# customink/lambdipy

Measured on NVIDIA H100. Metric: ELF-strip GB/s (build-tree .so bytes), higher is better.
Workload: dtype u8

## Files before the change

include/lambdipy_b200.h:

```cpp
#ifndef LAMBDIPY_B200_H
#define LAMBDIPY_B200_H
#include <stdint.h>
#ifdef __cplusplus
extern "C" {
#endif

typedef struct lb2_ctx lb2_ctx;

enum {
  LB2_OK = 0,
  LB2_E_CUDA = -1,
  LB2_E_ARG = -2,
  LB2_E_CAPACITY = -3,
  LB2_E_IO = -4,
  LB2_E_NODEVICE = -5,
  LB2_E_STATE = -6
};

enum {
  LB2_ST_OK = 0,
  LB2_ST_NOT_ELF = 1,
  LB2_ST_NOT_ELF64LE = 2,
  LB2_ST_BAD_TYPE = 3,
  LB2_ST_NO_SECTIONS = 4,
  LB2_ST_XINDEX = 5,
  LB2_ST_UNSUPPORTED_LAYOUT = 6,
  LB2_ST_BAD_NOTES = 7,
  LB2_ST_PLANNER_LIMIT = 8,
  LB2_ST_MALFORMED = -1
};

#define LB2_F_NO_MERGE_NOTES 1u

#define LB2_TREE_FALLBACK_HOST_STRIP 0x100u
#define LB2_TREE_TOLERATE_NON_ELF    0x200u
#define LB2_TREE_DRY_RUN             0x400u
#define LB2_TREE_CLEANUP             0x800u

typedef struct lb2_stats {
  uint32_t n_files, n_ok, n_unsupported, overflow;
  uint64_t in_bytes;
  uint64_t out_bytes;
  uint64_t copy_bytes;
  uint64_t header_bytes;
  uint64_t n_tiles;
  uint64_t out_bytes_needed;
  float plan_ms;
  float compact_ms;
  float h2d_ms, d2h_ms;
  uint64_t h2d_bytes;
  uint64_t d2h_bytes;
} lb2_stats;

typedef struct lb2_tree_stats {
  uint32_t n_selected;
  uint32_t n_gpu;
  uint32_t n_fallback;
  uint32_t n_skipped;
  uint32_t n_failed;
  uint32_t n_removed;
  uint64_t in_bytes, out_bytes;
  double walk_read_s;
  double gpu_s;
  double write_s;
  double fallback_s;
  double read_cpu_s;
  double write_cpu_s;
  double dma_wait_s;
  uint32_t io_threads, n_batches;
  lb2_stats batch;
} lb2_tree_stats;

int lb2_ctx_create(int device, lb2_ctx **ctx);
void lb2_ctx_destroy(lb2_ctx *ctx);
const char *lb2_last_error(const lb2_ctx *ctx);
const char *lb2_version(void);
int lb2_sm_count(const lb2_ctx *ctx);

void *lb2_dev_alloc(lb2_ctx *ctx, uint64_t bytes);
void lb2_dev_free(lb2_ctx *ctx, void *p);
void *lb2_pinned_alloc(lb2_ctx *ctx, uint64_t bytes);
void lb2_pinned_free(lb2_ctx *ctx, void *p);
int lb2_memcpy_h2d(lb2_ctx *ctx, void *d_dst, const void *h_src, uint64_t bytes);
int lb2_memcpy_d2h(lb2_ctx *ctx, void *h_dst, const void *d_src, uint64_t bytes);
int lb2_memset_d(lb2_ctx *ctx, void *d_dst, int value, uint64_t bytes);

int lb2_strip_device_async(lb2_ctx *ctx, const void *d_in, const uint64_t *h_in_off, const uint64_t *h_in_sizes,
                           uint32_t n_files, void *d_out, uint64_t out_capacity, uint32_t flags, void *stream);
int lb2_batch_results(lb2_ctx *ctx, uint64_t *h_out_off , uint64_t *h_out_sizes ,
                      int32_t *h_status , lb2_stats *stats);

typedef int (*lb2_chunk_fn)(void *user, uint32_t chunk, uint32_t first_file, uint32_t n_files, const void *d_out_slot,
                            const uint64_t *out_off, const uint64_t *out_sizes, const int32_t *status,
                            const lb2_stats *chunk_stats);
int lb2_strip_device_chunked(lb2_ctx *ctx, const void *d_in, const uint64_t *h_in_off, const uint64_t *h_in_sizes,
                             uint32_t n_files, void *d_out_ring, uint64_t slot_capacity, uint64_t max_chunk_bytes,
                             uint32_t flags, void *stream, lb2_chunk_fn on_chunk, void *user, uint64_t *h_out_sizes,
                             int32_t *h_status, lb2_stats *total);

int lb2_strip_host(lb2_ctx *ctx, const void *h_in, const uint64_t *h_in_off, const uint64_t *h_in_sizes,
                   uint32_t n_files, void *h_out, uint64_t out_capacity, uint64_t *h_out_off, uint64_t *h_out_sizes,
                   int32_t *h_status, uint32_t flags, lb2_stats *stats);

int lb2_strip_tree(lb2_ctx *ctx, const char *root, const char *suffix , uint32_t flags,
                   lb2_tree_stats *stats);
int lb2_strip_tree_ex(lb2_ctx *ctx, const char *root, const char *suffix, uint32_t flags, const char *keep_tests_regex,
                      lb2_tree_stats *stats);
int lb2_tree_cleanup(const char *root, const char *keep_tests_regex, uint32_t *n_removed);
int lb2_tree_prepare(lb2_ctx *ctx, uint64_t expected_tree_bytes);

int lb2_plan_device(lb2_ctx *ctx, const void *d_in, const uint64_t *h_in_off, const uint64_t *h_in_sizes,
                    uint32_t n_files, uint32_t flags, uint64_t *h_out_sizes, int32_t *h_status, lb2_stats *stats);

typedef struct lb2_fill_region {
  uint64_t offset;
  uint64_t len;
} lb2_fill_region;
int lb2_corpus_fill(lb2_ctx *ctx, void *d_arena, const lb2_fill_region *h_regions, uint32_t n_regions,
                    uint64_t seed, void *stream);

int lb2_corpus_scatter(lb2_ctx *ctx, void *d_arena, const void *h_data, uint64_t data_bytes, const uint64_t *h_dst,
                       const uint64_t *h_src, const uint64_t *h_len, uint32_t n);

#ifdef __cplusplus
}
#endif
#endif
```

lambdipy_b200/_native.py:

```python
import ctypes as C
import os

_HERE = os.path.dirname(os.path.abspath(__file__))
LIB_PATH = os.environ.get("LAMBDIPY_B200_LIB") or os.path.join(_HERE, "liblambdipy_b200.so")

LB2_OK, LB2_E_CUDA, LB2_E_ARG, LB2_E_CAPACITY, LB2_E_IO, LB2_E_NODEVICE, LB2_E_STATE = 0, -1, -2, -3, -4, -5, -6
ST_OK, ST_NOT_ELF, ST_NOT_ELF64LE, ST_BAD_TYPE, ST_NO_SECTIONS, ST_XINDEX = 0, 1, 2, 3, 4, 5
ST_UNSUPPORTED_LAYOUT, ST_BAD_NOTES, ST_PLANNER_LIMIT, ST_MALFORMED = 6, 7, 8, -1
F_NO_MERGE_NOTES = 1
TREE_FALLBACK_HOST_STRIP, TREE_TOLERATE_NON_ELF, TREE_DRY_RUN, TREE_CLEANUP = 0x100, 0x200, 0x400, 0x800

EXPORTS = [
    "lb2_ctx_create", "lb2_ctx_destroy", "lb2_last_error", "lb2_version", "lb2_sm_count",
    "lb2_dev_alloc", "lb2_dev_free", "lb2_pinned_alloc", "lb2_pinned_free",
    "lb2_memcpy_h2d", "lb2_memcpy_d2h", "lb2_memset_d",
    "lb2_strip_device_async", "lb2_batch_results", "lb2_strip_host", "lb2_strip_tree",
    "lb2_plan_device", "lb2_corpus_fill", "lb2_corpus_scatter",
    "lb2_strip_device_chunked", "lb2_tree_prepare", "lb2_strip_tree_ex", "lb2_tree_cleanup",
]


class Stats(C.Structure):
    _fields_ = [
        ("n_files", C.c_uint32), ("n_ok", C.c_uint32), ("n_unsupported", C.c_uint32), ("overflow", C.c_uint32),
        ("in_bytes", C.c_uint64), ("out_bytes", C.c_uint64), ("copy_bytes", C.c_uint64), ("header_bytes", C.c_uint64),
        ("n_tiles", C.c_uint64), ("out_bytes_needed", C.c_uint64),
        ("plan_ms", C.c_float), ("compact_ms", C.c_float), ("h2d_ms", C.c_float), ("d2h_ms", C.c_float),
        ("h2d_bytes", C.c_uint64), ("d2h_bytes", C.c_uint64),
    ]

    def as_dict(self):
        return {k: getattr(self, k) for k, _ in self._fields_}


class TreeStats(C.Structure):
    _fields_ = [
        ("n_selected", C.c_uint32), ("n_gpu", C.c_uint32), ("n_fallback", C.c_uint32), ("n_skipped", C.c_uint32),
        ("n_failed", C.c_uint32), ("n_removed", C.c_uint32),
        ("in_bytes", C.c_uint64), ("out_bytes", C.c_uint64),
        ("walk_read_s", C.c_double), ("gpu_s", C.c_double), ("write_s", C.c_double), ("fallback_s", C.c_double),
        ("read_cpu_s", C.c_double), ("write_cpu_s", C.c_double), ("dma_wait_s", C.c_double), ("io_threads", C.c_uint32), ("n_batches", C.c_uint32),
        ("batch", Stats),
    ]

    def as_dict(self):
        d = {k: getattr(self, k) for k, _ in self._fields_ if k != "batch"}
        d["batch"] = self.batch.as_dict()
        return d


class FillRegion(C.Structure):
    _fields_ = [("offset", C.c_uint64), ("len", C.c_uint64)]


class NativeError(RuntimeError):
    def __init__(self, code, msg):
        super().__init__("lambdipy_b200: rc=%d: %s" % (code, msg))
        self.code = code


class NoDeviceError(NativeError):
    pass


_lib = None


def load():
    global _lib
    if _lib is not None:
        return _lib
    if not os.path.exists(LIB_PATH):
        raise ImportError("%s is missing: run `python -m lambdipy_b200.build` (needs nvcc); "
                          "there is no CPU fallback for the strip path" % LIB_PATH)
    lib = C.CDLL(LIB_PATH)
    vp, u64p, i32p = C.c_void_p, C.POINTER(C.c_uint64), C.POINTER(C.c_int32)
    lib.lb2_ctx_create.argtypes = [C.c_int, C.POINTER(vp)]
    lib.lb2_ctx_create.restype = C.c_int
    lib.lb2_ctx_destroy.argtypes = [vp]
    lib.lb2_ctx_destroy.restype = None
    lib.lb2_last_error.argtypes = [vp]
    lib.lb2_last_error.restype = C.c_char_p
    lib.lb2_version.restype = C.c_char_p
    lib.lb2_sm_count.argtypes = [vp]
    lib.lb2_sm_count.restype = C.c_int
    lib.lb2_dev_alloc.argtypes = [vp, C.c_uint64]
    lib.lb2_dev_alloc.restype = vp
    lib.lb2_dev_free.argtypes = [vp, vp]
    lib.lb2_dev_free.restype = None
    lib.lb2_pinned_alloc.argtypes = [vp, C.c_uint64]
    lib.lb2_pinned_alloc.restype = vp
    lib.lb2_pinned_free.argtypes = [vp, vp]
    lib.lb2_pinned_free.restype = None
    lib.lb2_memcpy_h2d.argtypes = [vp, vp, vp, C.c_uint64]
    lib.lb2_memcpy_h2d.restype = C.c_int
    lib.lb2_memcpy_d2h.argtypes = [vp, vp, vp, C.c_uint64]
    lib.lb2_memcpy_d2h.restype = C.c_int
    lib.lb2_memset_d.argtypes = [vp, vp, C.c_int, C.c_uint64]
    lib.lb2_memset_d.restype = C.c_int
    lib.lb2_strip_device_async.argtypes = [vp, vp, u64p, u64p, C.c_uint32, vp, C.c_uint64, C.c_uint32, vp]
    lib.lb2_strip_device_async.restype = C.c_int
    lib.lb2_batch_results.argtypes = [vp, u64p, u64p, i32p, C.POINTER(Stats)]
    lib.lb2_batch_results.restype = C.c_int
    lib.lb2_strip_host.argtypes = [vp, vp, u64p, u64p, C.c_uint32, vp, C.c_uint64, u64p, u64p, i32p, C.c_uint32,
                                   C.POINTER(Stats)]
    lib.lb2_strip_host.restype = C.c_int
    lib.lb2_strip_tree.argtypes = [vp, C.c_char_p, C.c_char_p, C.c_uint32, C.POINTER(TreeStats)]
    lib.lb2_strip_tree.restype = C.c_int
    lib.lb2_plan_device.argtypes = [vp, vp, u64p, u64p, C.c_uint32, C.c_uint32, u64p, i32p, C.POINTER(Stats)]
    lib.lb2_plan_device.restype = C.c_int
    lib.lb2_corpus_fill.argtypes = [vp, vp, C.POINTER(FillRegion), C.c_uint32, C.c_uint64, vp]
    lib.lb2_corpus_fill.restype = C.c_int
    lib.lb2_corpus_scatter.argtypes = [vp, vp, vp, C.c_uint64, u64p, u64p, u64p, C.c_uint32]
    lib.lb2_corpus_scatter.restype = C.c_int
    lib.lb2_strip_device_chunked.argtypes = [vp, vp, u64p, u64p, C.c_uint32, vp, C.c_uint64, C.c_uint64, C.c_uint32, vp,
                                             vp, vp, u64p, i32p, C.POINTER(Stats)]
    lib.lb2_strip_device_chunked.restype = C.c_int
    lib.lb2_strip_tree_ex.argtypes = [vp, C.c_char_p, C.c_char_p, C.c_uint32, C.c_char_p, C.POINTER(TreeStats)]
    lib.lb2_strip_tree_ex.restype = C.c_int
    lib.lb2_tree_cleanup.argtypes = [C.c_char_p, C.c_char_p, C.POINTER(C.c_uint32)]
    lib.lb2_tree_cleanup.restype = C.c_int
    lib.lb2_tree_prepare.argtypes = [vp, C.c_uint64]
    lib.lb2_tree_prepare.restype = C.c_int
    _lib = lib
    return lib
# ... 67 lines not shown
```

lambdipy_b200/build.py:

```python
import os
import subprocess
import sys

HERE = os.path.dirname(os.path.abspath(__file__))
CSRC = os.path.join(HERE, "csrc")
OUT = os.path.join(HERE, "liblambdipy_b200.so")
SOURCES = ["plan.cu", "compact.cu", "compact_tma.cu", "corpus.cu", "api.cu"]
HEADERS = ["lb2_common.cuh", "copy_device.cuh", os.path.join("..", "..", "include", "lambdipy_b200.h")]
NVCC_FLAGS = [
    "-gencode", "arch=compute_90a,code=sm_90a", "-lineinfo", "-O3", "-std=c++17",
    "-Xcompiler", "-fPIC,-Wall,-Wno-unused-function", "--shared", "-cudart", "shared",
]


def needs_build():
    if not os.path.exists(OUT):
        return True
    t = os.path.getmtime(OUT)
    deps = [os.path.join(CSRC, s) for s in SOURCES + HEADERS] + [os.path.abspath(__file__)]
    return any(os.path.getmtime(d) > t for d in deps)


TIMING_OUT = os.path.join(HERE, "liblambdipy_b200_timing.so")


def build(force=False, verbose=False, timing=False):
    out = TIMING_OUT if timing else OUT
    if not timing and not force and not needs_build():
        return OUT
    nvcc = os.environ.get("NVCC", "/usr/local/cuda/bin/nvcc")
    cmd = [nvcc] + NVCC_FLAGS + (["-DLB2_PLAN_TIMING"] if timing else []) + (["-Xptxas", "-v"] if verbose else []) + \
        ["-o", out] + [os.path.join(CSRC, s) for s in SOURCES]
    r = subprocess.run(cmd, capture_output=True, text=True)
    if r.returncode != 0:
        sys.stderr.write(r.stdout + r.stderr)
        raise RuntimeError("nvcc failed building liblambdipy_b200.so")
    if verbose:
        sys.stderr.write(r.stdout + r.stderr)
    return out


if __name__ == "__main__":
    print(build(force="--force" in sys.argv, verbose="-v" in sys.argv, timing="--timing" in sys.argv))
```

lambdipy_b200/csrc/api.cu:

```cuda
#include "lb2_common.cuh"
#include "../../include/lambdipy_b200.h"

#include <algorithm>
#include <atomic>
#include <chrono>
#include <cctype>
#include <cerrno>
#include <cstdio>
#include <cstdlib>
#include <condition_variable>
#include <cstring>
#include <mutex>
#include <string>
#include <thread>
#include <vector>

#include <climits>
#include <dirent.h>
#include <regex.h>
#include <fcntl.h>
#include <spawn.h>
#include <sys/stat.h>
#include <sys/syscall.h>
#include <sys/wait.h>
// ... 767 lines not shown
    rmdir(p.c_str());
  } else {
    unlink(p.c_str());
  }
}

static void walk(const std::string &dir, const std::string &shown, bool top, const char *suffix, Cleanup *cl,
                 std::vector<TreeFile> &files, lb2_tree_stats *st) {
  DIR *d = opendir(dir.c_str());
  if (!d) return;
  std::vector<std::string> names;
  while (dirent *e = readdir(d))
    if (strcmp(e->d_name, ".") && strcmp(e->d_name, "..")) names.push_back(e->d_name);
  closedir(d);
  for (const std::string &name : names) {
    const std::string p = dir + "/" + name, line = shown + name;
    struct stat lsb, sb;
    if (lstat(p.c_str(), &lsb) != 0) continue;
    if (cl && cl->on) {
      bool remove = false;
      if (top && name[0] != '.' && (ends_with(name.c_str(), ".egg-info") || ends_with(name.c_str(), ".dist-info"))) remove = true;
      else if (name == "__pycache__") remove = true;
      else if (name == "tests" && line.find('\n') == std::string::npos &&
               !(cl->have_keep && regexec(&cl->keep, line.c_str(), 0, nullptr, 0) == 0)) remove = true;
      if (remove) { rm_rf(p); cl->n_removed++; continue; }
    }
    if (suffix && ends_with(name.c_str(), suffix)) {
      st->n_selected++;
      if (stat(p.c_str(), &sb) != 0 || !S_ISREG(sb.st_mode)) {
        st->n_failed++;
      } else {
        if (S_ISLNK(lsb.st_mode)) st->n_skipped++;
        files.push_back({p, (uint64_t)sb.st_size, sb.st_dev, sb.st_ino, 1});
      }
    }
    if (S_ISDIR(lsb.st_mode)) walk(p, line + "/", false, suffix, cl, files, st);
  }
}

static bool cleanup_init(Cleanup &cl, const char *keep_regex, std::string *err) {
  cl.on = true;
  if (keep_regex && *keep_regex) {
    if (regcomp(&cl.keep, keep_regex, REG_NOSUB) != 0) { if (err) *err = std::string("bad keep-tests pattern: ") + keep_regex; return false; }
    cl.have_keep = true;
  }
  return true;
}

static void dedupe(std::vector<TreeFile> &files) {
  std::sort(files.begin(), files.end(), [](const TreeFile &a, const TreeFile &b) {
    if (a.dev != b.dev) return a.dev < b.dev;
    if (a.ino != b.ino) return a.ino < b.ino;
    return a.path < b.path;
  });
  size_t w = 0;
  for (size_t i = 0; i < files.size(); i++) {
    if (w && files[w - 1].dev == files[i].dev && files[w - 1].ino == files[i].ino) files[w - 1].times++;
    else files[w++] = files[i];
  }
  files.resize(w);
  std::sort(files.begin(), files.end(), [](const TreeFile &a, const TreeFile &b) { return a.path < b.path; });
}

static int host_strip(const std::string &p) {
  const char *argv[] = {"strip", p.c_str(), nullptr};
  pid_t pid;
  if (posix_spawnp(&pid, "strip", nullptr, nullptr, const_cast<char *const *>(argv), environ) != 0) return 127;
  int status = 0;
  while (waitpid(pid, &status, 0) < 0 && errno == EINTR) {}
  return WIFEXITED(status) ? WEXITSTATUS(status) : 128;
}

template <class F> static void parallel_for(size_t n, int threads, F f) {
  std::atomic<size_t> next{0};
  std::vector<std::thread> pool;
  threads = (int)std::max<size_t>(1, std::min<size_t>((size_t)std::max(threads, 1), n));
  for (int t = 0; t < threads; t++)
    pool.emplace_back([&] { for (size_t i; (i = next.fetch_add(1)) < n;) f(i); });
  for (auto &th : pool) th.join();
}

struct Seg { uint32_t file; uint64_t file_off, len, slot_off; };
struct Slice { bool upload; uint8_t *dev; uint64_t len; uint32_t seg0, seg1; };

static void make_slices(bool upload, uint8_t *dev_base, const std::vector<uint32_t> &ids, const uint64_t *offs, const uint64_t *sizes,
                        uint64_t slot_bytes, std::vector<Seg> &segs, std::vector<Slice> &out) {
  const size_t m = ids.size();
  size_t k = 0;
  uint64_t c = 0;
  while (k < m) {
    if (sizes[k] == 0) { k++; c = 0; continue; }
    const uint64_t a = offs[k] + c, end = a + slot_bytes;
    Slice sl{upload, dev_base + a, 0, (uint32_t)segs.size(), 0};
    uint64_t last = a;
    while (k < m) {
      if (sizes[k] == 0) { k++; c = 0; continue; }
      const uint64_t fs = offs[k] + c, fe = offs[k] + sizes[k];
      if (fs >= end || fs - last > 65536) break;
      const uint64_t take = std::min(fe, end) - fs;
      segs.push_back({ids[k], c, take, fs - a});
      last = fs + take;
      if (last == fe) { k++; c = 0; } else { c += take; break; }
    }
    sl.seg1 = (uint32_t)segs.size();
    sl.len = last - a;
    out.push_back(sl);
  }
}

struct TreeWorker { cudaStream_t stream = nullptr; cudaEvent_t ev[2] = {nullptr, nullptr}; uint32_t k = 0; };

struct TreeEngine {
  uint8_t *h_ring = nullptr;
  uint64_t slot_bytes = 0;
  int n_workers = 0;
  std::vector<TreeWorker> workers;
  uint8_t *d_in[2] = {nullptr, nullptr}, *d_out[2] = {nullptr, nullptr};
  uint64_t cap_in[2] = {0, 0}, cap_out[2] = {0, 0};
};

static void tree_engine_free(TreeEngine *e) {
  if (!e) return;
  for (auto &w : e->workers) {
    if (w.stream) cudaStreamDestroy(w.stream);
    for (auto &ev : w.ev) if (ev) cudaEventDestroy(ev);
  }
  if (e->h_ring) cudaFreeHost(e->h_ring);
  for (int k = 0; k < 2; k++) { cudaFree(e->d_in[k]); cudaFree(e->d_out[k]); }
  delete e;
}

static int tree_engine_prepare(lb2_ctx *ctx, uint64_t expected_bytes) {
  if (ctx->tree) return LB2_OK;
  TreeEngine *e = new TreeEngine();
  e->slot_bytes = std::max<uint64_t>(1, env_u64("LB2_TREE_SLOT_MB", 4)) << 20;
  const unsigned hw = std::max(1u, std::thread::hardware_concurrency());
  int want = (int)env_u64("LB2_IO_THREADS", std::max(4u, std::min(32u, hw / 2)));
  want = std::max(want, 1);
  if (expected_bytes) want = (int)std::max<uint64_t>(2, std::min<uint64_t>((uint64_t)want, expected_bytes / (2 * e->slot_bytes) + 1));
  e->n_workers = want;
  NumaPreferred near_gpu(ctx->numa_node);
  cudaError_t err = cudaHostAlloc(&e->h_ring, (uint64_t)want * 2 * e->slot_bytes, cudaHostAllocDefault);
  if (err != cudaSuccess) { ctx->err = std::string("cudaHostAlloc(tree ring): ") + cudaGetErrorString(err); delete e; return LB2_E_CUDA; }
  e->workers.resize(want);
  for (auto &w : e->workers) {
    if (cudaStreamCreateWithFlags(&w.stream, cudaStreamNonBlocking) != cudaSuccess ||
        cudaEventCreateWithFlags(&w.ev[0], cudaEventDisableTiming) != cudaSuccess ||
        cudaEventCreateWithFlags(&w.ev[1], cudaEventDisableTiming) != cudaSuccess) {
      ctx->err = "cuda stream/event creation failed"; tree_engine_free(e); return LB2_E_CUDA;
    }
  }
  ctx->tree = e;
  return LB2_OK;
}

static bool pread_all(int fd, uint8_t *dst, uint64_t n, uint64_t off) {
  uint64_t got = 0;
  while (got < n) {
    ssize_t r = pread(fd, dst + got, n - got, (off_t)(off + got));
    if (r <= 0) { if (r < 0 && errno == EINTR) continue; return false; }
    got += (uint64_t)r;
  }
  return true;
}
static bool pwrite_all(int fd, const uint8_t *src, uint64_t n, uint64_t off) {
  uint64_t put = 0;
  while (put < n) {
    ssize_t r = pwrite(fd, src + put, n - put, (off_t)(off + put));
    if (r <= 0) { if (r < 0 && errno == EINTR) continue; return false; }
    put += (uint64_t)r;
  }
  return true;
}

extern "C" {

int lb2_tree_prepare(lb2_ctx *ctx, uint64_t expected_tree_bytes) {
  if (!ctx) return LB2_E_ARG;
  CK(cudaSetDevice(ctx->device));
  int rc = tree_engine_prepare(ctx, expected_tree_bytes);
  if (rc) return rc;
  rc = ws_reserve(ctx, ctx->ws, 256, 1 << 16);
  if (rc) return rc;
  return ws_reserve(ctx, ctx->ws2, 256, 1 << 16);
}

int lb2_tree_cleanup(const char *root, const char *keep_tests_regex, uint32_t *n_removed) {
  if (!root) return LB2_E_ARG;
  struct stat rsb;
  if (stat(root, &rsb) != 0 || !S_ISDIR(rsb.st_mode)) return LB2_E_IO;
  Cleanup cl;
  if (!cleanup_init(cl, keep_tests_regex, nullptr)) return LB2_E_ARG;
  std::string r = root;
  while (r.size() > 1 && r.back() == '/') r.pop_back();
  std::vector<TreeFile> files;
  lb2_tree_stats st;
  memset(&st, 0, sizeof st);
  walk(r, r + "/", true, nullptr, &cl, files, &st);
  if (cl.have_keep) regfree(&cl.keep);
  if (n_removed) *n_removed = cl.n_removed;
  return LB2_OK;
}

int lb2_strip_tree(lb2_ctx *ctx, const char *root, const char *suffix, uint32_t flags, lb2_tree_stats *st_out) {
  return lb2_strip_tree_ex(ctx, root, suffix, flags, nullptr, st_out);
}

int lb2_strip_tree_ex(lb2_ctx *ctx, const char *root, const char *suffix, uint32_t flags, const char *keep_tests_regex,
                      lb2_tree_stats *st_out) {
  if (!ctx || !root || !suffix) { if (ctx) ctx->err = "NULL argument"; return LB2_E_ARG; }
  CK(cudaSetDevice(ctx->device));
  lb2_tree_stats st;
  memset(&st, 0, sizeof st);
  double t0 = now_s();
  std::vector<TreeFile> files;
  struct stat rsb;
  if (stat(root, &rsb) != 0 || !S_ISDIR(rsb.st_mode)) { ctx->err = std::string("not a directory: ") + root; return LB2_E_IO; }
  std::string r = root;
  while (r.size() > 1 && r.back() == '/') r.pop_back();
  Cleanup cl;
  if ((flags & LB2_TREE_CLEANUP) && !cleanup_init(cl, keep_tests_regex, &ctx->err)) return LB2_E_ARG;
  walk(r, r + "/", true, suffix, &cl, files, &st);
  if (cl.have_keep) regfree(&cl.keep);
  st.n_removed = cl.n_removed;
  dedupe(files);
  const uint32_t n = (uint32_t)files.size();
  uint64_t tree_bytes = 0;
  for (auto &f : files) tree_bytes += f.size;
  st.walk_read_s = now_s() - t0;
  if (!n) { if (st_out) *st_out = st; return LB2_OK; }
  int rc = tree_engine_prepare(ctx, tree_bytes);
  if (rc) return rc;
  TreeEngine &E = *ctx->tree;
  const bool dry = (flags & LB2_TREE_DRY_RUN) != 0;

  const uint64_t batch_bytes = std::max<uint64_t>(1, env_u64("LB2_TREE_BATCH_MB", 1024)) << 20;
  struct Batch { uint32_t f0, f1; uint64_t span; };
  std::vector<Batch> batches;
  std::vector<uint64_t> off(n + 1), sizes(n), out_off(n + 1), out_sizes(n);
  std::vector<int32_t> status(n, LB2_ST_MALFORMED);
  for (uint32_t f = 0; f < n;) {
    uint64_t pos = 0;
    uint32_t g = f;
    while (g < n && (g == f || pos + ((files[g].size + 255) & ~255ull) <= batch_bytes)) {
      off[g] = pos; sizes[g] = files[g].size; pos += (files[g].size + 255) & ~255ull; g++;
    }
    batches.push_back({f, g, pos});
    f = g;
  }

  std::vector<Seg> segs;
  std::vector<Slice> queue;
  std::atomic<size_t> q_next{0}, q_done{0};
  size_t q_end = 0;
  std::mutex mu;
  std::condition_variable cv_work, cv_done;
  bool quit = false;
  std::atomic<int> io_fail{0};
  std::atomic<uint64_t> ns_read{0}, ns_write{0}, ns_dma{0};
  auto now_ns = [] { return (uint64_t)std::chrono::duration_cast<std::chrono::nanoseconds>(std::chrono::steady_clock::now().time_since_epoch()).count(); };
  std::vector<std::atomic<int>> read_bad(n), write_bad(n);
  std::vector<std::atomic<uint32_t>> segs_left(n);
  for (uint32_t i = 0; i < n; i++) { read_bad[i] = 0; write_bad[i] = 0; segs_left[i] = 0; }
  std::atomic<uint32_t> n_gpu{0}, n_failed{0}, n_skipped{0};
  std::atomic<uint64_t> in_b{0}, out_b{0};
  std::vector<uint64_t> final_size(n, 0);

  auto finish_file = [&](uint32_t i) {
    bool ok = write_bad[i] == 0;
    if (ok && final_size[i] != files[i].size) ok = truncate(files[i].path.c_str(), (off_t)final_size[i]) == 0;
    if (ok) { n_gpu++; in_b += files[i].size; out_b += final_size[i]; }
    else n_failed++;
  };
  auto run_slice = [&](TreeWorker &w, int widx, const Slice &sl) {
    uint8_t *slot = E.h_ring + ((uint64_t)widx * 2 + (w.k & 1)) * E.slot_bytes;
    cudaEvent_t ev = w.ev[w.k & 1];
    w.k++;
    if (sl.upload) {
      uint64_t t0 = now_ns();
      cudaEventSynchronize(ev);
      uint64_t t1 = now_ns();
      for (uint32_t q = sl.seg0; q < sl.seg1; q++) {
        const Seg &sg = segs[q];
        int fd = open(files[sg.file].path.c_str(), O_RDONLY | O_CLOEXEC);
        if (fd < 0 || !pread_all(fd, slot + sg.slot_off, sg.len, sg.file_off)) { read_bad[sg.file]++; io_fail++; }
        if (fd >= 0) close(fd);
      }
      uint64_t t2 = now_ns();
      cudaMemcpyAsync(sl.dev, slot, sl.len, cudaMemcpyHostToDevice, w.stream);
      cudaEventRecord(ev, w.stream);
      ns_dma += (t1 - t0) + (now_ns() - t2); ns_read += t2 - t1;
    } else {
      uint64_t t0 = now_ns();
      cudaMemcpyAsync(slot, sl.dev, sl.len, cudaMemcpyDeviceToHost, w.stream);
      cudaEventRecord(ev, w.stream);
      if (cudaEventSynchronize(ev) != cudaSuccess) io_fail++;
      uint64_t t1 = now_ns();
      ns_dma += t1 - t0;
      const uint64_t tw0 = t1;
      for (uint32_t q = sl.seg0; q < sl.seg1; q++) {
        const Seg &sg = segs[q];
        int fd = open(files[sg.file].path.c_str(), O_WRONLY | O_CLOEXEC);
        if (fd < 0 || !pwrite_all(fd, slot + sg.slot_off, sg.len, sg.file_off)) write_bad[sg.file]++;
        if (fd >= 0) close(fd);
        if (--segs_left[sg.file] == 0) finish_file(sg.file);
      }
      ns_write += now_ns() - tw0;
    }
  };
  std::vector<std::thread> pool;
  for (int wi = 0; wi < E.n_workers; wi++)
    pool.emplace_back([&, wi] {
      cudaSetDevice(ctx->device);
      TreeWorker &w = E.workers[wi];
      for (;;) {
        size_t idx;
        {
          std::unique_lock<std::mutex> lk(mu);
          cv_work.wait(lk, [&] { return quit || q_next.load() < q_end; });
          if (q_next.load() >= q_end) { if (quit) return; continue; }
          idx = q_next.fetch_add(1);
        }
        run_slice(w, wi, queue[idx]);
        if (q_done.fetch_add(1) + 1 == q_end) { std::lock_guard<std::mutex> lk(mu); cv_done.notify_all(); }
      }
    });
  auto submit_and_wait = [&](std::vector<Slice> &a, std::vector<Slice> &b) {
    {
      std::lock_guard<std::mutex> lk(mu);
      size_t i = 0, j = 0;
      while (i < a.size() || j < b.size()) {
        if (i < a.size()) queue.push_back(a[i++]);
        if (j < b.size()) queue.push_back(b[j++]);
      }
      q_end = queue.size();
    }
    cv_work.notify_all();
    std::unique_lock<std::mutex> lk(mu);
    cv_done.wait(lk, [&] { return q_done.load() >= q_end; });
  };
  auto stop_pool = [&] {
    { std::lock_guard<std::mutex> lk(mu); quit = true; }
    cv_work.notify_all();
    for (auto &th : pool) th.join();
  };

  auto upload_slices = [&](size_t bi, std::vector<Slice> &out) -> int {
    const Batch &b = batches[bi];
    const int set = (int)(bi & 1);
    if (E.cap_in[set] < b.span + 256) {
      cudaFree(E.d_in[set]); E.d_in[set] = nullptr; E.cap_in[set] = 0;
      const uint64_t need = b.span + 256;
      CK(cudaMalloc(&E.d_in[set], need));
      E.cap_in[set] = need;
    }
    std::vector<uint32_t> ids(b.f1 - b.f0);
    for (uint32_t i = b.f0; i < b.f1; i++) ids[i - b.f0] = i;
    make_slices(true, E.d_in[set], ids, off.data() + b.f0, sizes.data() + b.f0, E.slot_bytes, segs, out);
    return LB2_OK;
  };

  std::vector<void *> tmp_dev;
  std::vector<Slice> up, down, none;
  double t_gpu = 0, t_io0 = now_s();
  auto run_batches = [&]() -> int {
  int rc = upload_slices(0, up);
  if (rc == LB2_OK) submit_and_wait(up, none);
  for (size_t bi = 0; bi < batches.size() && rc == LB2_OK; bi++) {
    const Batch &b = batches[bi];
    const int set = (int)(bi & 1);
    const uint32_t m = b.f1 - b.f0;
    bool bad_read = false;
    for (uint32_t i = b.f0; i < b.f1; i++) bad_read |= read_bad[i] != 0;
    if (bad_read) { ctx->err = "could not read some selected files"; rc = LB2_E_IO; break; }
    const double tg = now_s();
    for (auto &w : E.workers) { CK(cudaStreamWaitEvent(ctx->stream, w.ev[0], 0)); CK(cudaStreamWaitEvent(ctx->stream, w.ev[1], 0)); }
    uint64_t want_out = b.span + (uint64_t)m * 4096 + (16u << 20);
    Workspace &ws = set ? ctx->ws2 : ctx->ws;
    lb2_stats bst;
    for (int attempt = 0; attempt < 2; attempt++) {
      if (E.cap_out[set] < want_out) {
        cudaFree(E.d_out[set]); E.d_out[set] = nullptr; E.cap_out[set] = 0;
        CK(cudaMalloc(&E.d_out[set], want_out));
        E.cap_out[set] = want_out;
      }
      rc = enqueue_batch(ctx, ws, E.d_in[set], off.data() + b.f0, sizes.data() + b.f0, m, E.d_out[set], E.cap_out[set], flags & 0xffu, ctx->stream, true);
      if (rc) break;
      rc = collect_batch(ctx, ws, out_off.data() + b.f0, out_sizes.data() + b.f0, status.data() + b.f0, &bst);
      if (rc != LB2_E_CAPACITY) break;
      want_out = bst.out_bytes_needed + (1u << 20);
    }
    if (rc) break;
    st.batch.n_files += m; st.batch.n_ok += bst.n_ok; st.batch.n_unsupported += bst.n_unsupported; st.batch.in_bytes += bst.in_bytes;
    st.batch.out_bytes += bst.out_bytes; st.batch.copy_bytes += bst.copy_bytes; st.batch.header_bytes += bst.header_bytes;
    st.batch.n_tiles += bst.n_tiles; st.batch.plan_ms += bst.plan_ms; st.batch.compact_ms += bst.compact_ms;
    std::vector<uint8_t *> src_base(m, E.d_out[set]);
    std::vector<uint64_t> src_off(out_off.begin() + b.f0, out_off.begin() + b.f1);
    for (uint32_t pass = 1; rc == LB2_OK; pass++) {
      std::vector<uint32_t> again;
      for (uint32_t i = b.f0; i < b.f1; i++) if (files[i].times > pass && status[i] == LB2_ST_OK) again.push_back(i);
      if (again.empty()) break;
      const uint32_t k2 = (uint32_t)again.size();
      std::vector<uint64_t> off2(k2 + 1), sz2(k2), ooff2(k2 + 1), osz2(k2);
      std::vector<int32_t> st2(k2);
      uint64_t p2 = 0;
      for (uint32_t k = 0; k < k2; k++) { off2[k] = p2; sz2[k] = out_sizes[again[k]]; p2 += (sz2[k] + 255) & ~255ull; }
      off2[k2] = p2;
      uint8_t *d_in2 = nullptr, *d_out2 = nullptr;
      const uint64_t cap2 = p2 + (uint64_t)k2 * 4096 + (64u << 20);
      CK(cudaMalloc(&d_in2, p2 + 256));
      tmp_dev.push_back(d_in2);
      CK(cudaMalloc(&d_out2, cap2));
      tmp_dev.push_back(d_out2);
      for (uint32_t k = 0; k < k2; k++) {
        const uint32_t i = again[k];
        CK(cudaMemcpyAsync(d_in2 + off2[k], src_base[i - b.f0] + src_off[i - b.f0], sz2[k], cudaMemcpyDeviceToDevice, ctx->stream));
      }
      lb2_stats b2;
      rc = enqueue_batch(ctx, ws, d_in2, off2.data(), sz2.data(), k2, d_out2, cap2, flags & 0xffu, ctx->stream, true);
      if (rc == LB2_OK) rc = collect_batch(ctx, ws, ooff2.data(), osz2.data(), st2.data(), &b2);
      if (rc == LB2_E_CAPACITY) { rc = LB2_OK; for (auto &x : st2) x = LB2_ST_UNSUPPORTED_LAYOUT; }
      if (rc) break;
      for (uint32_t k = 0; k < k2; k++) {
        const uint32_t i = again[k];
        status[i] = st2[k];
        if (st2[k] != LB2_ST_OK) continue;
        src_base[i - b.f0] = d_out2; src_off[i - b.f0] = ooff2[k]; out_sizes[i] = osz2[k];
      }
    }
    if (rc) break;
    t_gpu += now_s() - tg;
    down.clear(); up.clear();
    if (!dry) {
      std::vector<uint8_t *> bases;
      for (uint32_t i = 0; i < m; i++) if (std::find(bases.begin(), bases.end(), src_base[i]) == bases.end()) bases.push_back(src_base[i]);
      for (uint8_t *base : bases) {
        std::vector<std::pair<uint64_t, uint32_t>> ord;
        for (uint32_t i = 0; i < m; i++)
          if (src_base[i] == base && status[b.f0 + i] == LB2_ST_OK) ord.push_back({src_off[i], b.f0 + i});
        std::sort(ord.begin(), ord.end());
        std::vector<uint32_t> ids;
        std::vector<uint64_t> o2, s2;
        for (auto &pr : ord) { ids.push_back(pr.second); o2.push_back(pr.first); s2.push_back(out_sizes[pr.second]); }
        const size_t seg_before = segs.size();
        make_slices(false, base, ids, o2.data(), s2.data(), E.slot_bytes, segs, down);
        for (size_t q = seg_before; q < segs.size(); q++) segs_left[segs[q].file]++;
        for (auto &pr : ord) {
          final_size[pr.second] = out_sizes[pr.second];
          if (out_sizes[pr.second] == 0) finish_file(pr.second);
        }
      }
    } else {
      for (uint32_t i = b.f0; i < b.f1; i++) if (status[i] == LB2_ST_OK) { n_gpu++; in_b += files[i].size; out_b += out_sizes[i]; }
    }
    if (bi + 1 < batches.size()) rc = upload_slices(bi + 1, up);
    if (rc) break;
    submit_and_wait(down, up);
  }
  return rc;
  };
  rc = run_batches();
  stop_pool();
  cudaStreamSynchronize(ctx->stream);
  for (void *p : tmp_dev) cudaFree(p);
  st.gpu_s = t_gpu;
  st.read_cpu_s = ns_read.load() * 1e-9; st.write_cpu_s = ns_write.load() * 1e-9; st.dma_wait_s = ns_dma.load() * 1e-9;
  st.io_threads = (uint32_t)E.n_workers; st.n_batches = (uint32_t)batches.size();
  st.write_s = now_s() - t_io0 - t_gpu;
  if (rc) { if (st_out) *st_out = st; return rc; }

  t0 = now_s();
  std::vector<uint32_t> fallback;
  for (uint32_t i = 0; i < n; i++) if (status[i] != LB2_ST_OK) fallback.push_back(i);
  std::atomic<uint32_t> n_fb{0};
  parallel_for(fallback.size(), E.n_workers, [&](size_t k) {
    const uint32_t i = fallback[k];
    const bool non_elf = status[i] == LB2_ST_NOT_ELF;
    if (non_elf && (flags & LB2_TREE_TOLERATE_NON_ELF)) { n_skipped++; return; }
    if ((flags & LB2_TREE_FALLBACK_HOST_STRIP) && !dry) {
      bool ok = true;
      for (uint32_t q = 0; q < files[i].times && ok; q++) ok = host_strip(files[i].path) == 0;
      if (ok) n_fb++; else n_failed++;
    } else {
      n_failed++;
    }
  });
  st.fallback_s = now_s() - t0;
  st.n_gpu = n_gpu; st.n_fallback = n_fb; st.n_failed += n_failed; st.n_skipped += n_skipped;
  st.in_bytes = in_b; st.out_bytes = out_b;
  if (st_out) *st_out = st;
  return LB2_OK;
}

int lb2_corpus_fill(lb2_ctx *ctx, void *d_arena, const lb2_fill_region *h_regions, uint32_t n_regions, uint64_t seed, void *stream) {
  if (!ctx || !d_arena || (!h_regions && n_regions)) { if (ctx) ctx->err = "NULL argument"; return LB2_E_ARG; }
  CK(cudaSetDevice(ctx->device));
  cudaStream_t s = stream ? static_cast<cudaStream_t>(stream) : ctx->stream;
  if (!n_regions) return LB2_OK;
  std::vector<lb2_fill_region> pieces;
  const uint64_t P = 4ull << 20;
  for (uint32_t i = 0; i < n_regions; i++)
    for (uint64_t o = 0; o < h_regions[i].len; o += P) pieces.push_back({h_regions[i].offset + o, std::min(P, h_regions[i].len - o)});
  lb2_fill_region *d_regions = nullptr;
  CK(cudaMalloc(&d_regions, pieces.size() * sizeof(lb2_fill_region)));
  CK(cudaMemcpyAsync(d_regions, pieces.data(), pieces.size() * sizeof(lb2_fill_region), cudaMemcpyHostToDevice, s));
  launch_fill(static_cast<uint8_t *>(d_arena), reinterpret_cast<const FillRegion *>(d_regions), (uint32_t)pieces.size(), seed, ctx->sm_count * 8, s);
  CK(cudaStreamSynchronize(s));
  CK(cudaFree(d_regions));
  CK(cudaGetLastError());
  return LB2_OK;
}

int lb2_corpus_scatter(lb2_ctx *ctx, void *d_arena, const void *h_data, uint64_t data_bytes, const uint64_t *h_dst,
                       const uint64_t *h_src, const uint64_t *h_len, uint32_t n) {
  if (!ctx || !d_arena || (n && (!h_data || !h_dst || !h_src || !h_len))) { if (ctx) ctx->err = "NULL argument"; return LB2_E_ARG; }
  CK(cudaSetDevice(ctx->device));
  if (!n) return LB2_OK;
  cudaStream_t s = ctx->stream;
  uint8_t *d_stage = nullptr;
  CK(cudaMalloc(&d_stage, data_bytes + 256));
  CK(cudaMemcpyAsync(d_stage, h_data, data_bytes, cudaMemcpyHostToDevice, s));
  std::vector<Tile> tiles;
  for (uint32_t i = 0; i < n; i++)
    for (uint64_t o = 0; o < h_len[i]; o += TILE_BYTES) {
      Tile t;
      t.src = reinterpret_cast<uint64_t>(d_stage) + h_src[i] + o;
      t.dst_rel = h_dst[i] + o;
      t.len = (uint32_t)std::min<uint64_t>(TILE_BYTES, h_len[i] - o);
      t.file = 0;
      tiles.push_back(t);
    }
  Tile *d_tiles = nullptr;
  BatchCounters *d_ctr = nullptr;
  uint64_t *d_off = nullptr;
  CK(cudaMalloc(&d_tiles, tiles.size() * sizeof(Tile)));
  CK(cudaMalloc(&d_ctr, sizeof(BatchCounters)));
  CK(cudaMalloc(&d_off, sizeof(uint64_t)));
  BatchCounters c;
  memset(&c, 0, sizeof c);
  c.n_tiles = tiles.size();
  uint64_t zero = 0;
  CK(cudaMemcpyAsync(d_tiles, tiles.data(), tiles.size() * sizeof(Tile), cudaMemcpyHostToDevice, s));
  CK(cudaMemcpyAsync(d_ctr, &c, sizeof c, cudaMemcpyHostToDevice, s));
  CK(cudaMemcpyAsync(d_off, &zero, sizeof zero, cudaMemcpyHostToDevice, s));
  CompactArgs ca;
  ca.tiles = d_tiles; ca.ctr = d_ctr; ca.out_off = d_off; ca.out = static_cast<uint8_t *>(d_arena);
  ca.rebase_lo = ca.rebase_len = ca.rebase_delta = 0;
  launch_compact(ca, ctx->sm_count * 4, s);
  CK(cudaStreamSynchronize(s));
// ... 7 lines not shown
```

lambdipy_b200/csrc/lb2_common.cuh:

```cuda
#pragma once
#include <cstdint>
#include <cuda_runtime.h>

namespace lb2 {

struct Ehdr {
  uint8_t e_ident[16];
  uint16_t e_type, e_machine;
  uint32_t e_version;
  uint64_t e_entry, e_phoff, e_shoff;
  uint32_t e_flags;
  uint16_t e_ehsize, e_phentsize, e_phnum, e_shentsize, e_shnum, e_shstrndx;
};
struct Phdr {
  uint32_t p_type, p_flags;
  uint64_t p_offset, p_vaddr, p_paddr, p_filesz, p_memsz, p_align;
};
struct Shdr {
  uint32_t sh_name, sh_type;
  uint64_t sh_flags, sh_addr, sh_offset, sh_size;
  uint32_t sh_link, sh_info;
  uint64_t sh_addralign, sh_entsize;
};
static_assert(sizeof(Ehdr) == 64 && sizeof(Phdr) == 56 && sizeof(Shdr) == 64, "ELF64 layouts");
// ... 22 lines not shown
  ST_BAD_NOTES = 7,
  ST_PLANNER_LIMIT = 8,
  ST_MALFORMED = -1
};

constexpr int MAX_SH = 64;
constexpr int MAX_PH = 32;
constexpr int MAX_STR = 2048;
constexpr int MAX_NOTE_BYTES = 8192;
constexpr int MAX_NOTES = 320;
constexpr int MAX_EXT = 2 * MAX_SH + 12;

constexpr uint32_t SCR_EHDR = 0;
constexpr uint32_t SCR_STR = 64 + MAX_PH * 56;
constexpr uint32_t SCR_SHDR = SCR_STR + MAX_STR + 64;
constexpr uint32_t SCR_NOTES = SCR_SHDR + (MAX_SH + 1) * 64;
constexpr uint32_t SCR_STRIDE = ((SCR_NOTES + MAX_NOTE_BYTES + 255) / 256) * 256;

struct __align__(16) Tile {
  uint64_t src;
  uint64_t dst_rel;
  uint32_t len;
  uint32_t file;
};
static_assert(sizeof(Tile) == 32, "tile descriptors are read as two 16-byte vectors");
constexpr uint32_t TILE_BYTES = 16384;

struct BatchCounters {
  unsigned long long n_tiles;
  unsigned long long copy_bytes;
  unsigned long long out_bytes;
  unsigned long long header_bytes;
  unsigned long long in_bytes;
  unsigned int n_ok, n_unsupported;
  unsigned int overflow;
  unsigned int pad;
  unsigned long long claim_bulk;
  unsigned long long claim_help;
  unsigned int n_ranges, ranges_overflow;
  unsigned int n_big, pad2;
};

struct PlanArgs {
  const uint8_t *in;
  const uint64_t *in_off;
  const uint64_t *in_size;
  uint32_t n_files;
  uint32_t flags;
  uint8_t *scratch;
  uint64_t *out_size;
  int32_t *status;
  Tile *tiles;
  uint64_t tile_cap;
  BatchCounters *ctr;
  struct UpRange *up_ranges;
  uint32_t up_cap;
  struct BigExt *big;
  uint32_t big_cap;
};
struct UpRange { uint64_t off, len; };
struct BigExt { uint64_t src, dst, len, tile_index; uint32_t file, pad; };
constexpr uint32_t BIG_EXT_TILES = 512;
constexpr uint32_t BIG_PART_TILES = 2048;
__host__ __device__ inline Tile extent_tile(uint64_t src, uint64_t dst, uint64_t len, uint32_t file, uint32_t k) {
  const uint64_t t0 = dst / TILE_BYTES;
  uint64_t b = (t0 + k) * TILE_BYTES, e = b + TILE_BYTES;
  if (b < dst) b = dst;
  if (e > dst + len) e = dst + len;
  Tile t;
  t.src = src ? src + (b - dst) : 0;
  t.dst_rel = b;
  t.len = (uint32_t)(e - b);
  t.file = file;
  return t;
}
struct CompactArgs {
  const Tile *tiles;
  BatchCounters *ctr;
  const uint64_t *out_off;
  uint8_t *out;
  uint64_t rebase_lo, rebase_len, rebase_delta;
};
struct FillRegion { uint64_t offset, len; };

void launch_plan(const PlanArgs &a, cudaStream_t s);
void launch_scan(const uint64_t *out_size, uint64_t *out_off, uint32_t n, uint64_t out_cap, BatchCounters *ctr, const BigExt *big,
                 uint32_t big_cap, Tile *tiles, int expand_ctas, cudaStream_t s);
void launch_compact(const CompactArgs &a, int grid, cudaStream_t s);
void launch_compact_tma(const CompactArgs &a, int grid, cudaStream_t s);
void launch_fill(uint8_t *arena, const FillRegion *d_regions, uint32_t n, uint64_t seed, int grid, cudaStream_t s);

}
```

Measured before the change: 2581.

## Write back only dirty 4KiB pages by diffing stripped output against original on GPU

Adds a GPU kernel that compares each stripped file against its original bytes page by page and marks the pages that differ. The host then builds write runs only over dirty pages, merging small gaps, and pwrites just those ranges into the file in place. The aim is to cut device-to-host transfer and file write volume when stripping changes few pages. In exchange it adds an extra kernel launch, a stream synchronize and a flag copy per batch. It also relies on the file still holding the original bytes, and the file must be truncated to the new size elsewhere.

New measurement: 2581, median of 6. About the same (+0.0%).

```diff
diff --git a/include/lambdipy_b200.h b/include/lambdipy_b200.h
--- a/include/lambdipy_b200.h
+++ b/include/lambdipy_b200.h
@@ -69,6 +69,7 @@
   double dma_wait_s;
   uint32_t io_threads, n_batches;
   lb2_stats batch;
+  uint64_t write_bytes;
 } lb2_tree_stats;
 
 int lb2_ctx_create(int device, lb2_ctx **ctx);
diff --git a/lambdipy_b200/_native.py b/lambdipy_b200/_native.py
--- a/lambdipy_b200/_native.py
+++ b/lambdipy_b200/_native.py
@@ -40,7 +40,7 @@
         ("in_bytes", C.c_uint64), ("out_bytes", C.c_uint64),
         ("walk_read_s", C.c_double), ("gpu_s", C.c_double), ("write_s", C.c_double), ("fallback_s", C.c_double),
         ("read_cpu_s", C.c_double), ("write_cpu_s", C.c_double), ("dma_wait_s", C.c_double), ("io_threads", C.c_uint32), ("n_batches", C.c_uint32),
-        ("batch", Stats),
+        ("batch", Stats), ("write_bytes", C.c_uint64),
     ]
 
     def as_dict(self):
diff --git a/lambdipy_b200/build.py b/lambdipy_b200/build.py
--- a/lambdipy_b200/build.py
+++ b/lambdipy_b200/build.py
@@ -5,7 +5,7 @@
 HERE = os.path.dirname(os.path.abspath(__file__))
 CSRC = os.path.join(HERE, "csrc")
 OUT = os.path.join(HERE, "liblambdipy_b200.so")
-SOURCES = ["plan.cu", "compact.cu", "compact_tma.cu", "corpus.cu", "api.cu"]
+SOURCES = ["plan.cu", "compact.cu", "compact_tma.cu", "corpus.cu", "dirty.cu", "api.cu"]
 HEADERS = ["lb2_common.cuh", "copy_device.cuh", os.path.join("..", "..", "include", "lambdipy_b200.h")]
 NVCC_FLAGS = [
     "-gencode", "arch=compute_90a,code=sm_90a", "-lineinfo", "-O3", "-std=c++17",
diff --git a/lambdipy_b200/csrc/api.cu b/lambdipy_b200/csrc/api.cu
--- a/lambdipy_b200/csrc/api.cu
+++ b/lambdipy_b200/csrc/api.cu
@@ -873,23 +873,26 @@
 
 struct Seg { uint32_t file; uint64_t file_off, len, slot_off; };
 struct Slice { bool upload; uint8_t *dev; uint64_t len; uint32_t seg0, seg1; };
-
-static void make_slices(bool upload, uint8_t *dev_base, const std::vector<uint32_t> &ids, const uint64_t *offs, const uint64_t *sizes,
-                        uint64_t slot_bytes, std::vector<Seg> &segs, std::vector<Slice> &out) {
-  const size_t m = ids.size();
+struct Piece { uint32_t file; uint64_t dev_off, file_off, len; };
+constexpr uint64_t RUN_GAP_PAGES = 4;
+
+static void make_slices(bool upload, uint8_t *dev_base, const std::vector<Piece> &pieces, uint64_t slot_bytes, std::vector<Seg> &segs,
+                        std::vector<Slice> &out) {
+  const size_t m = pieces.size();
   size_t k = 0;
   uint64_t c = 0;
   while (k < m) {
-    if (sizes[k] == 0) { k++; c = 0; continue; }
-    const uint64_t a = offs[k] + c, end = a + slot_bytes;
+    if (pieces[k].len == 0) { k++; c = 0; continue; }
+    const uint64_t a = pieces[k].dev_off + c, end = a + slot_bytes;
     Slice sl{upload, dev_base + a, 0, (uint32_t)segs.size(), 0};
     uint64_t last = a;
     while (k < m) {
-      if (sizes[k] == 0) { k++; c = 0; continue; }
-      const uint64_t fs = offs[k] + c, fe = offs[k] + sizes[k];
+      const Piece &pc = pieces[k];
+      if (pc.len == 0) { k++; c = 0; continue; }
+      const uint64_t fs = pc.dev_off + c, fe = pc.dev_off + pc.len;
       if (fs >= end || fs - last > 65536) break;
       const uint64_t take = std::min(fe, end) - fs;
-      segs.push_back({ids[k], c, take, fs - a});
+      segs.push_back({pc.file, pc.file_off + c, take, fs - a});
       last = fs + take;
       if (last == fe) { k++; c = 0; } else { c += take; break; }
     }
@@ -908,6 +911,10 @@
   std::vector<TreeWorker> workers;
   uint8_t *d_in[2] = {nullptr, nullptr}, *d_out[2] = {nullptr, nullptr};
   uint64_t cap_in[2] = {0, 0}, cap_out[2] = {0, 0};
+  DirtyFile *d_dfiles = nullptr;
+  uint8_t *d_dirty = nullptr, *h_dirty = nullptr;
+  uint32_t cap_dfiles = 0;
+  uint64_t cap_dirty = 0;
 };
 
 static void tree_engine_free(TreeEngine *e) {
@@ -918,6 +925,8 @@
   }
   if (e->h_ring) cudaFreeHost(e->h_ring);
   for (int k = 0; k < 2; k++) { cudaFree(e->d_in[k]); cudaFree(e->d_out[k]); }
+  cudaFree(e->d_dfiles); cudaFree(e->d_dirty);
+  if (e->h_dirty) cudaFreeHost(e->h_dirty);
   delete e;
 }
 
@@ -1054,7 +1063,7 @@
   std::vector<std::atomic<uint32_t>> segs_left(n);
   for (uint32_t i = 0; i < n; i++) { read_bad[i] = 0; write_bad[i] = 0; segs_left[i] = 0; }
   std::atomic<uint32_t> n_gpu{0}, n_failed{0}, n_skipped{0};
-  std::atomic<uint64_t> in_b{0}, out_b{0};
+  std::atomic<uint64_t> in_b{0}, out_b{0}, wr_b{0};
   std::vector<uint64_t> final_size(n, 0);
 
   auto finish_file = [&](uint32_t i) {
@@ -1093,6 +1102,7 @@
         const Seg &sg = segs[q];
         int fd = open(files[sg.file].path.c_str(), O_WRONLY | O_CLOEXEC);
         if (fd < 0 || !pwrite_all(fd, slot + sg.slot_off, sg.len, sg.file_off)) write_bad[sg.file]++;
+        else wr_b += sg.len;
         if (fd >= 0) close(fd);
         if (--segs_left[sg.file] == 0) finish_file(sg.file);
       }
@@ -1145,9 +1155,9 @@
       CK(cudaMalloc(&E.d_in[set], need));
       E.cap_in[set] = need;
     }
-    std::vector<uint32_t> ids(b.f1 - b.f0);
-    for (uint32_t i = b.f0; i < b.f1; i++) ids[i - b.f0] = i;
-    make_slices(true, E.d_in[set], ids, off.data() + b.f0, sizes.data() + b.f0, E.slot_bytes, segs, out);
+    std::vector<Piece> whole(b.f1 - b.f0);
+    for (uint32_t i = b.f0; i < b.f1; i++) whole[i - b.f0] = {i, off[i], 0, sizes[i]};
+    make_slices(true, E.d_in[set], whole, E.slot_bytes, segs, out);
     return LB2_OK;
   };
 
@@ -1220,6 +1230,37 @@
       }
     }
     if (rc) break;
+    std::vector<uint64_t> page0(m, 0);
+    if (!dry) {
+      std::vector<DirtyFile> df;
+      uint64_t n_pages = 0;
+      for (uint32_t i = 0; i < m; i++) {
+        if (status[b.f0 + i] != LB2_ST_OK) continue;
+        page0[i] = n_pages;
+        df.push_back({src_base[i] + src_off[i], E.d_in[set] + off[b.f0 + i], out_sizes[b.f0 + i], sizes[b.f0 + i], n_pages});
+        n_pages += (out_sizes[b.f0 + i] + DIRTY_PAGE - 1) / DIRTY_PAGE;
+      }
+      if (n_pages) {
+        if (E.cap_dfiles < df.size()) {
+          cudaFree(E.d_dfiles); E.d_dfiles = nullptr; E.cap_dfiles = 0;
+          CK(cudaMalloc(&E.d_dfiles, df.size() * sizeof(DirtyFile)));
+          E.cap_dfiles = (uint32_t)df.size();
+        }
+        if (E.cap_dirty < n_pages) {
+          cudaFree(E.d_dirty); E.d_dirty = nullptr;
+          if (E.h_dirty) cudaFreeHost(E.h_dirty);
+          E.h_dirty = nullptr; E.cap_dirty = 0;
+          CK(cudaMalloc(&E.d_dirty, n_pages));
+          CK(cudaHostAlloc(&E.h_dirty, n_pages, cudaHostAllocDefault));
+          E.cap_dirty = n_pages;
+        }
+        CK(cudaMemcpyAsync(E.d_dfiles, df.data(), df.size() * sizeof(DirtyFile), cudaMemcpyHostToDevice, ctx->stream));
+        launch_dirty_pages(E.d_dfiles, (uint32_t)df.size(), n_pages, E.d_dirty, ctx->sm_count * 8, ctx->stream);
+        CK(cudaGetLastError());
+        CK(cudaMemcpyAsync(E.h_dirty, E.d_dirty, n_pages, cudaMemcpyDeviceToHost, ctx->stream));
+        CK(cudaStreamSynchronize(ctx->stream));
+      }
+    }
     t_gpu += now_s() - tg;
     down.clear(); up.clear();
     if (!dry) {
@@ -1230,11 +1271,26 @@
         for (uint32_t i = 0; i < m; i++)
           if (src_base[i] == base && status[b.f0 + i] == LB2_ST_OK) ord.push_back({src_off[i], b.f0 + i});
         std::sort(ord.begin(), ord.end());
-        std::vector<uint32_t> ids;
-        std::vector<uint64_t> o2, s2;
-        for (auto &pr : ord) { ids.push_back(pr.second); o2.push_back(pr.first); s2.push_back(out_sizes[pr.second]); }
+        std::vector<Piece> runs;
+        for (auto &pr : ord) {
+          const uint32_t f = pr.second;
+          const uint64_t size = out_sizes[f], np = (size + DIRTY_PAGE - 1) / DIRTY_PAGE;
+          const uint8_t *flag = E.h_dirty + page0[f - b.f0];
+          for (uint64_t p = 0; p < np;) {
+            if (p && !flag[p]) {
+              const void *nx = memchr(flag + p, 1, np - p);
+              if (!nx) break;
+              p = (uint64_t)(static_cast<const uint8_t *>(nx) - flag);
+            }
+            uint64_t q = p + 1;
+            for (uint64_t r = q; r < np && r - q <= RUN_GAP_PAGES; r++) if (flag[r]) q = r + 1;
+            const uint64_t s = p * DIRTY_PAGE, e = std::min<uint64_t>(q * DIRTY_PAGE, size);
+            runs.push_back({f, pr.first + s, s, e - s});
+            p = q;
+          }
+        }
         const size_t seg_before = segs.size();
-        make_slices(false, base, ids, o2.data(), s2.data(), E.slot_bytes, segs, down);
+        make_slices(false, base, runs, E.slot_bytes, segs, down);
         for (size_t q = seg_before; q < segs.size(); q++) segs_left[segs[q].file]++;
         for (auto &pr : ord) {
           final_size[pr.second] = out_sizes[pr.second];
@@ -1256,6 +1312,7 @@
   for (void *p : tmp_dev) cudaFree(p);
   st.gpu_s = t_gpu;
   st.read_cpu_s = ns_read.load() * 1e-9; st.write_cpu_s = ns_write.load() * 1e-9; st.dma_wait_s = ns_dma.load() * 1e-9;
+  st.write_bytes = wr_b;
   st.io_threads = (uint32_t)E.n_workers; st.n_batches = (uint32_t)batches.size();
   st.write_s = now_s() - t_io0 - t_gpu;
   if (rc) { if (st_out) *st_out = st; return rc; }
diff --git a/lambdipy_b200/csrc/dirty.cu b/lambdipy_b200/csrc/dirty.cu
--- /dev/null
+++ b/lambdipy_b200/csrc/dirty.cu
@@ -0,0 +1,58 @@
+#include "lb2_common.cuh"
+
+namespace lb2 {
+
+__device__ __forceinline__ uint32_t first_page_file(const DirtyFile *files, uint32_t n, uint64_t page) {
+  uint32_t lo = 0, hi = n;
+  while (hi - lo > 1) {
+    const uint32_t mid = (lo + hi) / 2;
+    if (files[mid].page0 <= page) lo = mid; else hi = mid;
+  }
+  return lo;
+}
+
+__global__ void __launch_bounds__(256) lb2_dirty_pages_kernel(const DirtyFile *files, uint32_t n_files, uint64_t n_pages, uint8_t *dirty) {
+  const int lane = threadIdx.x & 31;
+  const uint64_t warps = (uint64_t)gridDim.x * (blockDim.x >> 5);
+  for (uint64_t p = (uint64_t)blockIdx.x * (blockDim.x >> 5) + (threadIdx.x >> 5); p < n_pages; p += warps) {
+    const DirtyFile f = files[first_page_file(files, n_files, p)];
+    const uint64_t b = (p - f.page0) * DIRTY_PAGE;
+    const uint64_t e = b + DIRTY_PAGE < f.out_size ? b + DIRTY_PAGE : f.out_size;
+    bool diff = e > f.orig_size;
+    if (!diff) {
+      const uint4 *o = reinterpret_cast<const uint4 *>(f.out + b), *s = reinterpret_cast<const uint4 *>(f.orig + b);
+      const uint32_t n16 = (uint32_t)((e - b + 15) / 16);
+      uint4 x[DIRTY_PAGE / 512], y[DIRTY_PAGE / 512];
+#pragma unroll
+      for (int k = 0; k < DIRTY_PAGE / 512; k++) {
+        const uint32_t v = lane + 32 * k;
+        if (v < n16) { x[k] = __ldg(o + v); y[k] = __ldg(s + v); }
+        else x[k] = y[k] = make_uint4(0, 0, 0, 0);
+      }
+#pragma unroll
+      for (int k = 0; k < DIRTY_PAGE / 512; k++) {
+        const uint32_t v = lane + 32 * k;
+        uint32_t d[4] = {x[k].x ^ y[k].x, x[k].y ^ y[k].y, x[k].z ^ y[k].z, x[k].w ^ y[k].w};
+        const uint64_t valid = e - b - 16ull * v;
+        if (v < n16 && valid < 16) {
+#pragma unroll
+          for (int w = 0; w < 4; w++) {
+            const int keep = (int)valid - 4 * w;
+            d[w] &= keep >= 4 ? 0xffffffffu : keep <= 0 ? 0u : (1u << (8 * keep)) - 1u;
+          }
+        }
+        diff |= (d[0] | d[1] | d[2] | d[3]) != 0;
+      }
+    }
+    diff = __any_sync(0xffffffffu, diff);
+    if (lane == 0) dirty[p] = diff ? 1 : 0;
+  }
+}
+
+void launch_dirty_pages(const DirtyFile *files, uint32_t n_files, uint64_t n_pages, uint8_t *dirty, int grid, cudaStream_t s) {
+  if (!n_pages) return;
+  const uint64_t need = (n_pages + 7) / 8;
+  lb2_dirty_pages_kernel<<<(int)(need < (uint64_t)grid ? need : (uint64_t)grid), 256, 0, s>>>(files, n_files, n_pages, dirty);
+}
+
+}
diff --git a/lambdipy_b200/csrc/lb2_common.cuh b/lambdipy_b200/csrc/lb2_common.cuh
--- a/lambdipy_b200/csrc/lb2_common.cuh
+++ b/lambdipy_b200/csrc/lb2_common.cuh
@@ -128,6 +128,11 @@
   uint64_t rebase_lo, rebase_len, rebase_delta;
 };
 struct FillRegion { uint64_t offset, len; };
+struct DirtyFile {
+  const uint8_t *out, *orig;
+  uint64_t out_size, orig_size, page0;
+};
+constexpr uint32_t DIRTY_PAGE = 4096;
 
 void launch_plan(const PlanArgs &a, cudaStream_t s);
 void launch_scan(const uint64_t *out_size, uint64_t *out_off, uint32_t n, uint64_t out_cap, BatchCounters *ctr, const BigExt *big,
@@ -135,5 +140,6 @@
 void launch_compact(const CompactArgs &a, int grid, cudaStream_t s);
 void launch_compact_tma(const CompactArgs &a, int grid, cudaStream_t s);
 void launch_fill(uint8_t *arena, const FillRegion *d_regions, uint32_t n, uint64_t seed, int grid, cudaStream_t s);
+void launch_dirty_pages(const DirtyFile *files, uint32_t n_files, uint64_t n_pages, uint8_t *dirty, int grid, cudaStream_t s);
 
 }
```
